# 0xWOLAND/zkvm-pairings

Hardware: AMD Instinct MI355X
Metric: BLS12-381 pairings/s on 2^20 random (G1,G2) pairs; bit-exact Gt vs ref (CPU oracle: the reference's pairings.rs is empty) (higher is better)
Workload: dtype u32

## Files before the change

### zkvm_pairings_amd/csrc/zkp_coop.hip

```cpp
#include "zkp_coop.hpp"
#include "zkp_plan.hpp"
#include "zkp_msm_plan.hpp"

#include <cstdio>
#include <cstdlib>
#include <cstring>
#include <vector>

#include "zkp_coop_prog.inc"
#include "zkp_fp28.hpp"
#include "zkp_coop_mulacc.inc"
#include "zkp_prep_dbl.inc"
#include "zkp_valid_steps.inc"

using namespace zkp28;

namespace {

constexpr int GROUPS = 5;
constexpr int LIG = ZKP_COOP_G;
constexpr int ST_SIZE = ZKP_COOP_ST_SIZE;
constexpr int NLINES = ZKP_COOP_NLINES;
static_assert(zkp::plan::NLINES == NLINES && zkp::plan::ST_SIZE == ST_SIZE && zkp::plan::GROUPS == GROUPS,
              "zkp_plan.hpp (the host's planning arithmetic, checked under sanitizers on the CPU) follows the generated programs");
// ... 6 lines not shown

struct NDev { const uint32_t* cnt; uint32_t base; };
__device__ __forceinline__ uint32_t eff_n(uint32_t n, const NDev& nd) {
    if (!nd.cnt) return n;
    const uint32_t m = *nd.cnt;
    const uint32_t left = m > nd.base ? m - nd.base : 0u;
    return left < n ? left : n;
}

struct CoopArgs {
    const uint32_t* hdr;
    const uint32_t* tbl;
    const uint4* rtbl;
    const int4* consts;
    const int4* lines;
    int4* state;
    const uint64_t* wire_in;
    uint64_t* wire_out;
    uint8_t* ok;
    int* all_ok;
    uint32_t n_checks;
    uint32_t nc;
    uint32_t k;
    uint32_t S;
    uint32_t nconst;
    uint32_t st_off;
    uint32_t chk_off;
    NDev nd;
};

__device__ __forceinline__ void lds_ld(int32_t* x, const int4* lds, int off, int S) {
// ... 162 lines not shown
                    const uint64_t* src = A.wire_in + ((size_t)check + (arg == K_WIRE2 ? A.chk_off : 0u)) * 72 + idx * 6;
                    uint64_t ww[6];
#pragma unroll
                    for (int i = 0; i < 6; i++) ww[i] = src[i];
#pragma unroll
                    for (int i = 0; i < NL; i++) {
                        const int bit = W * i, word = bit >> 6, sh = bit & 63;
                        uint64_t v = ww[word] >> sh;
                        if (sh > 64 - W && word + 1 < 6) v |= ww[word + 1] << (64 - sh);
                        x[i] = (int32_t)(v & (uint64_t)MASK);
                    }
                } else {
                    size_t rec;
                    if (arg == K_LINE) rec = ((size_t)cursor * A.k * 6 + pair6 + idx) * n_checks + check;
                    else rec = (size_t)(idx + A.st_off) * A.nc + check;
                    const int4* src = (arg == K_LINE ? A.lines : (const int4*)A.state) + rec * 4;
                    int4 v0 = src[0], v1 = src[1], v2 = src[2], v3 = src[3];
                    x[0] = v0.x; x[1] = v0.y; x[2] = v0.z; x[3] = v0.w; x[4] = v1.x; x[5] = v1.y; x[6] = v1.z; x[7] = v1.w;
                    x[8] = v2.x; x[9] = v2.y; x[10] = v2.z; x[11] = v2.w; x[12] = v3.x; x[13] = v3.y;
                }
                lds_st(lds, gbase + (int)(w & 63), PS, x);
            }
            cursor += h1;
        } else if (op == OP_GSTORE) {
            const uint32_t w = tbl[off + lig];
            const uint32_t idx = w >> 8;
            const bool part = active && ((w >> 7) & 1);
            int32_t x[NL];
            lds_ld(x, lds, gbase + (int)(w & 63), PS);
            if (arg == K_STATE) {
                if (part) {
                    int4* dst = A.state + ((size_t)(idx + A.st_off) * A.nc + check) * 4;
                    dst[0] = make_int4(x[0], x[1], x[2], x[3]);
                    dst[1] = make_int4(x[4], x[5], x[6], x[7]);
                    dst[2] = make_int4(x[8], x[9], x[10], x[11]);
                    dst[3] = make_int4(x[12], x[13], 0, 0);
                }
            } else {
                uint32_t f[NL];
                canon28(f, x);
                if (part && A.wire_out) {
                    uint64_t o[6] = {0, 0, 0, 0, 0, 0};
#pragma unroll
                    for (int i = 0; i < NL; i++) {
                        const int bit = W * i, word = bit >> 6, sh = bit & 63;
                        o[word] |= (uint64_t)f[i] << sh;
                        if (sh > 64 - W && word + 1 < 6) o[word + 1] |= (uint64_t)f[i] >> (64 - sh);
                    }
                    uint64_t* dst = A.wire_out + (size_t)check * 72 + idx * 6;
#pragma unroll
                    for (int i = 0; i < 6; i++) dst[i] = o[i];
// ... 74 lines not shown
}

__device__ __forceinline__ void ksq_forms(int32_t* xr, int32_t* xi, int32_t* yr, int32_t* yi, bool a_lane, bool v_mine) {
    if (a_lane) {
#pragma unroll
        for (int i = 0; i < NL; i++) {
            const int32_t tr = xr[i] + yr[i], ti = xi[i] + yi[i];
            const int32_t vr = v_mine ? xr[i] : yr[i], vi = v_mine ? xi[i] : yi[i];
            xr[i] = tr;
            xi[i] = ti;
            yr[i] = vi - tr;
            yi[i] = -ti - vr;
        }
    }
}
__global__ void __launch_bounds__(64, KSQ_WAVES) k_ksq(int4* state, uint32_t n_checks_in, uint32_t nc, uint32_t elem_in, uint32_t elem_snap,
                                                           uint32_t nsq, uint64_t snap_mask, NDev nd) {
    extern __shared__ int4 parked[];
    const uint32_t n_checks = eff_n(n_checks_in, nd);
    if (blockIdx.x * KS_CHECKS >= n_checks) return;
    const int lane = threadIdx.x;
    const int r = lane & 3;
    const bool b_lane = r & 1;
    const bool mine_is_v = r == 0 || r == 3;
    const uint32_t check_raw = blockIdx.x * KS_CHECKS + (lane >> 2);
    const bool active = check_raw < n_checks;
    const uint32_t check = active ? check_raw : n_checks - 1;
    const int tu = (r & 2) ? 1 : 3, tv = (r & 2) ? 5 : 2;
    int4* const st = state + (size_t)check * 4;
    auto rec = [&](uint32_t e) -> int4* { return st + (size_t)e * nc * 4; };

    int32_t xr[NL], xi[NL], yr[NL], yi[NL];
    {
        Fp28 u0, u1, v0, v1;
        rec_load(u0, rec(elem_in + 2 * tu));
        rec_load(u1, rec(elem_in + 2 * tu + 1));
        rec_load(v0, rec(elem_in + 2 * tv));
        rec_load(v1, rec(elem_in + 2 * tv + 1));
        const Fp28 &m0 = mine_is_v ? v0 : u0, &m1 = mine_is_v ? v1 : u1, &o0 = mine_is_v ? u0 : v0, &o1 = mine_is_v ? u1 : v1;
        park_st(parked, lane, m0.l, m1.l);
#pragma unroll
        for (int i = 0; i < NL; i++) { xr[i] = m0.l[i]; xi[i] = m1.l[i]; yr[i] = o0.l[i]; yi[i] = o1.l[i]; }
        ksq_forms(xr, xi, yr, yi, !b_lane, r == 0);
    }
    uint32_t snap = elem_snap;
// ... 8 lines not shown
    for (uint32_t it = 0; it < nsq; it++) {
        {
            constexpr uint32_t PL[NL] = {ZKP28_P_LIMBS};
            asm volatile(ZKP_KSQ_BODY_ASM
                         : ZKP_KSQ_BODY_IO(xr, xi, yr, yi)
                         : [p0] "s"(PL[0]), [p1] "s"(PL[1]), [p2] "s"(PL[2]), [p3] "s"(PL[3]), [p4] "s"(PL[4]), [p5] "s"(PL[5]), [p6] "s"(PL[6]),
                           [p7] "s"(PL[7]), [p8] "s"(PL[8]), [p9] "s"(PL[9]), [p10] "s"(PL[10]), [p11] "s"(PL[11]), [p12] "s"(PL[12]),
                           [p13] "s"(PL[13]), [pinv] "s"(ZKP28_PINV)
                         : ZKP_KSQ_BODY_CLOBBERS);
        }
        int l_ = lane;
        asm volatile("" : "+v"(l_));
        const bool a_lane = !(l_ & 1), v_mine = (l_ & 3) == 0;
        if (it < 64 && ((snap_mask >> it) & 1)) {
            const uint32_t chk_ = blockIdx.x * KS_CHECKS + (l_ >> 2);
            int4* const st_ = state + (size_t)(chk_ < n_checks ? chk_ : n_checks - 1) * 4;
            auto rec_ = [&](uint32_t e) -> int4* { return st_ + (size_t)e * nc * 4; };
            const int tu_ = (l_ & 2) ? 1 : 3, tv_ = (l_ & 2) ? 5 : 2;
            if (chk_ < n_checks && a_lane) {
                Fp28 o;
#pragma unroll
                for (int i = 0; i < NL; i++) o.l[i] = xr[i];
                rec_store(rec_(snap + 2 * (v_mine ? tv_ : tu_)), o);
#pragma unroll
                for (int i = 0; i < NL; i++) o.l[i] = xi[i];
                rec_store(rec_(snap + 2 * (v_mine ? tv_ : tu_) + 1), o);
#pragma unroll
                for (int i = 0; i < NL; i++) o.l[i] = yr[i];
                rec_store(rec_(snap + 2 * (v_mine ? tu_ : tv_)), o);
#pragma unroll
                for (int i = 0; i < NL; i++) o.l[i] = yi[i];
                rec_store(rec_(snap + 2 * (v_mine ? tu_ : tv_) + 1), o);
// ... 787 lines not shown
    acc_mul(acc, o.l, o.l);
    Fp28 nrm;
    acc_reduce(nrm.l, acc);
    Fp28 ninv = f_inv(nrm);
    Fp28 zi = f_mul_v(c ? c_neg(p.z) : p.z, ninv);
    Fp28 zi2 = f.sqr(zi);
    Fp28 ax = f.mul(p.x, zi2), ay = f.mul(p.y, f.mul(zi2, zi));
    if (inf) { f_zero(ax); ay = f.one(); }
    if (live) {
        fp28_to_wire(out + 24 * (size_t)i + 6 * c, ax);
        fp28_to_wire(out + 24 * (size_t)i + 12 + 6 * c, ay);
        if (out_inf && c == 0) out_inf[i] = inf ? 1 : 0;
    }
}

__global__ void __launch_bounds__(64) k_batch_inv(int4* state, uint32_t n_checks_in, uint32_t nc, uint32_t Bf, uint32_t elem_n, uint32_t elem_ninv,
                                                  uint32_t count, NDev nd) {
    const uint32_t n_checks = eff_n(n_checks_in, nd);
    const uint32_t B = Bf & 0x7fffffffu;
    const bool fermat = Bf >> 31;
    const uint32_t total = n_checks * count;
    const uint32_t L = (total + B - 1) / B;
    const uint32_t i = blockIdx.x * 64 + threadIdx.x;
    if (i >= L) return;
    auto recno = [&](uint32_t idx) -> size_t { const uint32_t j = idx / n_checks; return ((size_t)j * nc + (idx - j * n_checks)) * 4; };
    int4* N = state + (size_t)elem_n * nc * 4;
    int4* I = state + (size_t)elem_ninv * nc * 4;
    Fp28 acc = f_const(K28_ONE);
    uint32_t cnt = 0;
    Fp28 e_next;
    rec_load(e_next, N + recno(i));
#pragma unroll 1
    for (uint32_t idx = i; idx < total && cnt < B; idx += L, cnt++) {
        Fp28 e = e_next;
        if (idx + L < total && cnt + 1 < B) rec_load(e_next, N + recno(idx + L));
        if (B > 1) {
            rec_store(I + recno(idx), acc);
            if (f_is_zero(e)) e = f_const(K28_ONE);
            fp28_mul(acc, acc, e);
        } else {
            acc = e;
        }
// ... 13 lines not shown
        if (j) {
            const size_t nx = recno(i + (j - 1) * L);
            rec_load(e_next, N + nx);
            rec_load(pre_next, I + nx);
        }
        if (f_is_zero(e)) {
            f_zero(r);
        } else {
            fp28_mul(r, inv, pre);
            fp28_mul(inv, inv, e);
        }
        rec_store(I + at, r);
    }
}

__global__ void __launch_bounds__(64, 2) k_kdec_a(int4* state, uint32_t n_checks_in, uint32_t nc, uint32_t elem_snap, uint32_t count, uint32_t elem_n,
                                                  NDev nd) {
    const uint32_t n_checks = eff_n(n_checks_in, nd);
    if (blockIdx.x * 32u >= n_checks * count) return;
    const uint32_t tid = blockIdx.x * 64 + threadIdx.x;
    const int c = (int)(tid & 1);
    uint32_t e = tid >> 1;
    bool live = e < n_checks * count;
    if (!live) e = n_checks * count - 1;
    const uint32_t sn = e / n_checks, check = e - sn * n_checks;
    int4* const st = state + (size_t)check * 4;
    const uint32_t base = elem_snap + 12 * sn;
    auto rec = [&](uint32_t el) -> int4* { return st + (size_t)el * nc * 4; };
    F2 f{c};
    Fp28 z2, z3, z4, z5;
    rec_load(z2, rec(base + 6 + c));
    rec_load(z3, rec(base + 4 + c));
    rec_load(z4, rec(base + 2 + c));
    rec_load(z5, rec(base + 10 + c));
    const bool z2_zero = f.is_zero(z2);
    Fp28 s5 = f.sqr(z5), o;
    swap_pair(o, s5);
    Fp28 na = c ? c_add(o, s5) : c_sub(s5, o);
    Fp28 s4 = f.sqr(z4);
    na = c_sub(c_add(na, c_add(c_dbl(s4), s4)), c_dbl(z3));
    Fp28 nb = na;
    if (__any(z2_zero)) nb = c_dbl(f.mul(z4, z5));
    Fp28 N = z2_zero ? nb : na, D = z2_zero ? z3 : z2;
    swap_pair(o, D);
    Acc acc;
    acc_zero(acc);
    acc_mul(acc, D.l, D.l);
    acc_mul(acc, o.l, o.l);
    Fp28 n;
    acc_reduce(n.l, acc);
    if (!z2_zero) n = c_dbl(c_dbl(n));
    if (live) {
        int4* dn = rec(base + 8 + c);
        dn[0] = make_int4(N.l[0], N.l[1], N.l[2], N.l[3]);
        dn[1] = make_int4(N.l[4], N.l[5], N.l[6], N.l[7]);
        dn[2] = make_int4(N.l[8], N.l[9], N.l[10], N.l[11]);
        dn[3] = make_int4(N.l[12], N.l[13], z2_zero ? 1 : 0, 0);
        if (c == 0) rec_store(rec(elem_n + sn), n);
    }
}
__global__ void __launch_bounds__(64, 3) k_kdec_b(int4* state, uint32_t n_checks_in, uint32_t nc, uint32_t elem_snap, uint32_t count, uint32_t elem_ninv,
                                                  NDev nd) {
    const uint32_t n_checks = eff_n(n_checks_in, nd);
    if (blockIdx.x * 32u >= n_checks * count) return;
    const uint32_t tid = blockIdx.x * 64 + threadIdx.x;
    const int c = (int)(tid & 1);
    uint32_t e = tid >> 1;
    bool live = e < n_checks * count;
    if (!live) e = n_checks * count - 1;
    const uint32_t sn = e / n_checks, check = e - sn * n_checks;
    int4* const st = state + (size_t)check * 4;
    const uint32_t base = elem_snap + 12 * sn;
    auto rec = [&](uint32_t el) -> int4* { return st + (size_t)el * nc * 4; };
    F2 f{c};
    Fp28 N, D, ninv, z2, z3;
    int d_is_z3;
    {
        const int4* sn_ = rec(base + 8 + c);
        const int4 v0 = sn_[0], v1 = sn_[1], v2 = sn_[2], v3 = sn_[3];
        N.l[0] = v0.x; N.l[1] = v0.y; N.l[2] = v0.z; N.l[3] = v0.w; N.l[4] = v1.x; N.l[5] = v1.y; N.l[6] = v1.z; N.l[7] = v1.w;
        N.l[8] = v2.x; N.l[9] = v2.y; N.l[10] = v2.z; N.l[11] = v2.w; N.l[12] = v3.x; N.l[13] = v3.y;
        d_is_z3 = v3.z;
    }
    rec_load(z2, rec(base + 6 + c));
    rec_load(ninv, rec(elem_ninv + sn));
    D = z2;
    if (__any(d_is_z3 != 0)) {
        Fp28 z3e;
        rec_load(z3e, rec(base + 4 + c));
#pragma unroll
        for (int i = 0; i < NL; i++) D.l[i] = d_is_z3 ? z3e.l[i] : z2.l[i];
    }
    Fp28 dinv = f_mul_v(c ? c_neg(D) : D, ninv);
    Fp28 z1 = f.mul(N, dinv);
    Fp28 t;
    {
        Acc acc;
        acc_zero(acc);
        auto mulacc = [&](const Fp28& a, const Fp28& b, int k) {
            Fp28 ao, bo;
            swap_pair(ao, a);
            swap_pair(bo, b);
            int32_t x1[NL], x2[NL];
#pragma unroll
// ... 5 lines not shown
            acc_mul(acc, x2, bo.l);
        };
        {
            Fp28 o1;
            swap_pair(o1, z1);
            int32_t x[NL], y[NL];
#pragma unroll
            for (int i = 0; i < NL; i++) {
                x[i] = 2 * (o1.l[i] + (c ? o1.l[i] : z1.l[i]));
                y[i] = z1.l[i] - (c ? 0 : o1.l[i]);
            }
            acc_mul(acc, x, y);
        }
        {
            Fp28 z5;
            rec_load(z5, rec(base + 10 + c));
            mulacc(z2, z5, 1);
        }
        {
            Fp28 z4;
            rec_load(z3, rec(base + 4 + c));
            rec_load(z4, rec(base + 2 + c));
            mulacc(z3, z4, -3);
        }
        acc_reduce(t.l, acc);
    }
    Fp28 o;
    swap_pair(o, t);
    Fp28 z0 = c ? c_add(o, t) : c_add(c_sub(t, o), f_const(K28_ONE));
    z0 = f_vred(z0);
    if (live) {
        rec_store(rec(base + c), z0);
        rec_store(rec(base + 8 + c), z1);
    }
}

__global__ void k_fp28_op(int op, const uint64_t* a, const uint64_t* b, size_t n, uint64_t* out) {
    size_t i = (size_t)blockIdx.x * blockDim.x + threadIdx.x;
    if (i >= n) return;
    Fp28 x, y, r;
    fp28_from_wire(x, a + 6 * i);
    if (op <= 2) fp28_from_wire(y, b + 6 * i);
    switch (op) {
        case 0: fp28_mul(r, x, y); break;
        case 1: f_add(r, x, y); break;
        case 2: f_sub(r, x, y); break;
        case 3: r = c_neg(x); break;
        case 4: fp28_mul(r, x, x); break;
// ... 348 lines not shown
        if (out_inf && c == 0) out_inf[sg] = inf ? 1 : 0;
    }
}

__global__ void __launch_bounds__(64) k_primer() {}

}

namespace zkp {

struct CoopProgDev { uint32_t* hdr; uint32_t* tbl; uint4* rtbl; uint32_t nslot; uint32_t nconst; uint32_t wide; };
constexpr int MAX_PIPES = plan::MAX_PIPES;
struct CoopDev;
struct CoopPipe {
    int4* lines;  size_t lines_bytes;
    int4* state;  size_t state_bytes;
    hipStream_t stream;
    hipEvent_t done;
    CoopDev* owner;
    NDev nd;
};
struct CoopDev {
    CoopProgDev progs[ZKP_PROG_COUNT];
    int4* consts;
    CoopPipe pipe[MAX_PIPES];
    plan::Knobs kn;
    bool inv_fermat;
    int cus;
    bool prime_now;
    int prime;
    int4* big_state;
    size_t big_state_bytes;
    int4* vscratch;
    size_t vscratch_bytes;
    hipEvent_t ready;
    struct ProfEv { int cls; hipEvent_t a, b; };
    std::vector<ProfEv>* prof;
    bool prof_phase_c;
    const uint32_t* n_dev;
};

enum { PRIME_PREP, PRIME_KSQ, PRIME_INV };
enum { PROF_PREP = 0, PROF_MILLER, PROF_FEXP_A, PROF_INV, PROF_KSQ, PROF_KDEC_A, PROF_KDEC_B, PROF_C_DEEP, PROF_C_PLAIN, PROF_CLASSES };
struct ProfScope {
    CoopDev* d; hipStream_t s; hipEvent_t b = nullptr;
    ProfScope(CoopDev* d_, hipStream_t s_, int cls) : d(d_), s(s_) {
// ... 103 lines not shown
    if (d->vscratch) (void)hipFree(d->vscratch);
    for (int i = 0; i < MAX_PIPES; i++) {
        if (d->pipe[i].lines) (void)hipFree(d->pipe[i].lines);
        if (d->pipe[i].state) (void)hipFree(d->pipe[i].state);
        if (d->pipe[i].stream) (void)hipStreamDestroy(d->pipe[i].stream);
        if (d->pipe[i].done) (void)hipEventDestroy(d->pipe[i].done);
    }
    if (d->ready) (void)hipEventDestroy(d->ready);
    delete d;
    st->d_prog = nullptr;
    st->available = false;
}

bool coop_selected(const CoopState* st, int kind) { return st->available && kind != 1; }

static hipError_t ensure_buf(int4** p, size_t* cap, size_t bytes) {
    if (bytes <= *cap) return hipSuccess;
    if (*p) { hipError_t e = hipFree(*p); if (e != hipSuccess) return e; *p = nullptr; *cap = 0; }
    hipError_t e = hipMalloc((void**)p, bytes);
    if (e == hipSuccess) { *cap = bytes; zkp_dbg_alloc("coop.buf", *p, bytes); }
    return e;
}

static hipError_t prime(const CoopDev* d, hipStream_t s, size_t blocks, int cls) {
    if (!d || !d->prime || d->cus <= 0 || !blocks || !d->prime_now) return hipSuccess;
    const size_t c = (size_t)d->cus;
    const bool band = cls == PRIME_KSQ ? (blocks > 3 * c && blocks <= 4 * c) || (blocks > 6 * c && blocks <= 8 * c)
                                       : (blocks > 2 * c && blocks <= 3 * c);
    if (!(band || (d->prime >= 2 && blocks > c && blocks <= 12 * c))) return hipSuccess;
    hipLaunchKernelGGL(k_primer, dim3((unsigned)blocks), dim3(64), 0, s);
    return hipGetLastError();
// ... 102 lines not shown
                return e;
        }
    }
    return hipSuccess;
}

template <class Body>
static hipError_t for_chunks(CoopDev* d, size_t n_total, size_t k, bool need_lines, bool need_state, hipStream_t s, Body body, size_t chunk_override = 0) {
    if (!n_total) return hipSuccess;
    hipError_t e;
    const plan::Chunks pc = plan::plan_chunks(d->kn, n_total, k, need_lines, chunk_override, d->prof != nullptr);
    const size_t chunk = pc.chunk;
    const int pipes = pc.pipes;
    for (int i = 0; i < pipes; i++) {
        if (need_lines && (e = ensure_buf(&d->pipe[i].lines, &d->pipe[i].lines_bytes, plan::lines_bytes(plan::group_size(d->kn, k), pc.cmax))) != hipSuccess) return e;
        if (need_state && (e = ensure_buf(&d->pipe[i].state, &d->pipe[i].state_bytes, plan::state_bytes(pc.cmax))) != hipSuccess) return e;
    }
    if ((e = hipEventRecord(d->ready, s)) != hipSuccess) return e;
    for (int i = 0; i < pipes; i++)
        if ((e = hipStreamWaitEvent(d->pipe[i].stream, d->ready, 0)) != hipSuccess) return e;
    int c = 0;
    for (size_t base = 0; base < n_total; base += chunk, c++) {
        uint32_t n = (uint32_t)((n_total - base) < chunk ? (n_total - base) : chunk);
        if ((e = body(&d->pipe[c % pipes], base, n)) != hipSuccess) return e;
    }
    for (int i = 0; i < pipes; i++) {
        if ((e = hipEventRecord(d->pipe[i].done, d->pipe[i].stream)) != hipSuccess) return e;
        if ((e = hipStreamWaitEvent(s, d->pipe[i].done, 0)) != hipSuccess) return e;
    }
    return hipSuccess;
}

hipError_t coop_miller(CoopState* st, const uint64_t* g1, const uint64_t* g2, const uint8_t* i1, const uint8_t* i2, size_t n_checks, size_t k,
                       uint64_t* out, hipStream_t s) {
    CoopDev* d = (CoopDev*)st->d_prog;
    if (!coop_supports_k(k)) return hipErrorNotSupported;
    d->prime_now = n_checks <= d->kn.chunk;
    return for_chunks(d, n_checks, k, true, true, s, [&](CoopPipe* pp, size_t base, uint32_t n) -> hipError_t {
        return miller_on_pipe(d, pp, g1, g2, i1, i2, base, n, n, k, out + 72 * base);
    });
}

static hipError_t run_ksq(hipStream_t s, int4* state, uint32_t n_checks, uint32_t nc, uint32_t elem_in, uint32_t elem_snap, uint32_t nsq,
                          uint64_t snap_mask, CoopDev* d = nullptr, NDev nd = NDev{nullptr, 0}) {
    if (!n_checks || !nsq) return hipSuccess;
    if (snap_mask && nsq > 64) return hipErrorInvalidValue;
    { hipError_t ep = prime(d, s, (n_checks + KS_CHECKS - 1) / KS_CHECKS, PRIME_KSQ); if (ep != hipSuccess) return ep; }
    ProfScope prof(d, s, PROF_KSQ);
    hipLaunchKernelGGL(k_ksq, dim3((n_checks + KS_CHECKS - 1) / KS_CHECKS), dim3(64), 7 * 64 * sizeof(int4), s, state, n_checks, nc, elem_in, elem_snap, nsq, snap_mask, nd);
    return hipGetLastError();
}

static hipError_t run_inv(CoopDev* d, hipStream_t s, int4* state, uint32_t n, uint32_t nc, uint32_t elem_n, uint32_t elem_ninv, uint32_t count,
                          NDev nd = NDev{nullptr, 0}) {
    const size_t total = (size_t)n * count;
    if (!total) return hipSuccess;
    const plan::Inv pi = plan::plan_inv(d->kn, n, count);
    const uint32_t B = pi.batch;
    const size_t lanes = pi.lanes;
    { hipError_t ep = prime(d, s, (lanes + 63) / 64, PRIME_INV); if (ep != hipSuccess) return ep; }
    ProfScope prof(d, s, PROF_INV);
    hipLaunchKernelGGL(k_batch_inv, dim3((unsigned)((lanes + 63) / 64)), dim3(64), 0, s, state, n, nc, B | (d->inv_fermat ? 0x80000000u : 0u), elem_n,
                       elem_ninv, count, nd);
    return hipGetLastError();
}

static hipError_t run_fexp_c(CoopDev* d, CoopPipe* pp, uint32_t n, uint32_t nc, uint64_t* wire_out, uint8_t* ok, int* all_ok) {
    hipError_t e;
// ... 26 lines not shown
                e = hipErrorInvalidValue;
        }
        if (e != hipSuccess) break;
    }
    d->prof_phase_c = false;
    return e;
}

template <class PhaseA>
static hipError_t two_phase(CoopDev* d, size_t n_total, size_t k, bool need_lines, hipStream_t s, uint64_t* out, uint8_t* ok, int* all_ok,
                            PhaseA phase_a) {
    hipError_t e;
    for (size_t sb = 0; sb < n_total; sb += d->kn.super) {
        const size_t ns = n_total - sb < d->kn.super ? n_total - sb : d->kn.super;
        d->prime_now = ns <= d->kn.chunk && n_total <= d->kn.chunk;
        if ((e = ensure_buf(&d->big_state, &d->big_state_bytes, plan::state_bytes(ns))) != hipSuccess) return e;
        e = for_chunks(d, ns, k, need_lines, false, s, [&](CoopPipe* pp, size_t base, uint32_t n) -> hipError_t {
            CoopPipe v = *pp;
            v.state = d->big_state + 4 * base;
            v.nd = NDev{d->n_dev, (uint32_t)(sb + base)};
            return phase_a(&v, sb + base, n, (uint32_t)ns);
        });
        if (e != hipSuccess) return e;
        if ((e = run_inv(d, s, d->big_state, (uint32_t)ns, (uint32_t)ns, ZKP_COOP_ST_N, ZKP_COOP_ST_NINV, 1, NDev{d->n_dev, (uint32_t)sb})) != hipSuccess) return e;
        const plan::PhaseC pcc = plan::plan_phase_c(d->kn, ns, d->prof != nullptr);
        if (pcc.mode == plan::C_PARTS) {
            const size_t part = pcc.part;
            e = for_chunks(d, ns, 1, false, false, s, [&](CoopPipe* pp, size_t base, uint32_t n) -> hipError_t {
                CoopPipe v = *pp;
                v.state = d->big_state + 4 * base;
                v.nd = NDev{d->n_dev, (uint32_t)(sb + base)};
                return run_fexp_c(d, &v, n, (uint32_t)ns, out ? out + 72 * (sb + base) : nullptr, ok ? ok + sb + base : nullptr, all_ok);
            }, part);
        } else {
            CoopPipe v = d->pipe[0];
            v.state = d->big_state;
            v.stream = s;
            v.nd = NDev{d->n_dev, (uint32_t)sb};
            e = run_fexp_c(d, &v, (uint32_t)ns, (uint32_t)ns, out ? out + 72 * sb : nullptr, ok ? ok + sb : nullptr, all_ok);
        }
        if (e != hipSuccess) return e;
    }
    return hipSuccess;
}

// ... 70 lines not shown
            int one = -1, pa = -1, pb = -1;
            switch (op) {
                case 13: pa = ZKP_PROG_TW_FP2_INV_A; pb = ZKP_PROG_TW_FP2_INV_B; break;
                case 14: one = ZKP_PROG_TW_FP2_NR; break;
                case 15: one = ZKP_PROG_TW_FP2_MULFP; break;
                case 16: one = ZKP_PROG_TW_FP6_BY1; break;
                case 17: one = ZKP_PROG_TW_FP6_BY01; break;
                case 18: one = ZKP_PROG_TW_FP6_NR; break;
                case 19: pa = ZKP_PROG_TW_FP6_INV_A; pb = ZKP_PROG_TW_FP6_INV_B; break;
                default: pa = ZKP_PROG_FEXP_A_WIRE; pb = ZKP_PROG_TW_FP12_INV_B; break;
            }
            if (one >= 0) {
                if ((e = run_prog(d, &v, one, m, m, 1, ab + 72 * base, out + 72 * base, nullptr, nullptr, 0, (uint32_t)n)) != hipSuccess) return e;
                continue;
            }
            if ((e = ensure_buf(&d->pipe[0].state, &d->pipe[0].state_bytes, plan::state_bytes(d->kn.chunk))) != hipSuccess) return e;
            v.state = d->pipe[0].state;
            if ((e = run_prog(d, &v, pa, m, m, 1, ab + 72 * base, nullptr, nullptr, nullptr)) != hipSuccess) return e;
            if ((e = run_inv(d, s, v.state, m, m, ZKP_COOP_ST_N, ZKP_COOP_ST_NINV, 1)) != hipSuccess) return e;
            if ((e = run_prog(d, &v, pb, m, m, 1, nullptr, out + 72 * base, nullptr, nullptr)) != hipSuccess) return e;
            continue;
        }
        if (op <= 10) {
            if ((e = run_prog(d, &v, progs[op], m, m, 1, ab + 72 * base, out + 72 * base, nullptr, nullptr, 0, (uint32_t)n)) != hipSuccess) return e;
            if (op == 4 && (e = hipMemset2DAsync(out + 72 * base + 36, 576, 0, 288, m, s)) != hipSuccess) return e;
            continue;
        }
        if (op == 11 && (repeat < 1 || repeat > 64)) return hipErrorInvalidValue;
        if ((e = ensure_buf(&d->pipe[0].state, &d->pipe[0].state_bytes, plan::state_bytes(d->kn.chunk))) != hipSuccess) return e;
        v.state = d->pipe[0].state;
        if (op == 12) {
            if ((e = run_prog(d, &v, ZKP_PROG_TW_TO_SNAP, m, m, 1, ab + 72 * base, nullptr, nullptr, nullptr)) != hipSuccess) return e;
        } else {
            if ((e = run_prog(d, &v, ZKP_PROG_TW_TO_STATE, m, m, 1, ab + 72 * base, nullptr, nullptr, nullptr)) != hipSuccess) return e;
            if ((e = run_ksq(s, v.state, m, m, 0, ZKP_COOP_ST_SNAP, repeat, 1ull << (repeat - 1), d)) != hipSuccess) return e;
        }
        hipLaunchKernelGGL(k_kdec_a, dim3((2 * m + 63) / 64), dim3(64), 0, s, v.state, m, m, (uint32_t)ZKP_COOP_ST_SNAP, 1u, (uint32_t)ZKP_COOP_ST_KN, NDev{nullptr, 0});
        if ((e = hipGetLastError()) != hipSuccess) return e;
        if ((e = run_inv(d, s, v.state, m, m, ZKP_COOP_ST_KN, ZKP_COOP_ST_KNINV, 1)) != hipSuccess) return e;
        hipLaunchKernelGGL(k_kdec_b, dim3((2 * m + 63) / 64), dim3(64), 0, s, v.state, m, m, (uint32_t)ZKP_COOP_ST_SNAP, 1u, (uint32_t)ZKP_COOP_ST_KNINV, NDev{nullptr, 0});
        if ((e = hipGetLastError()) != hipSuccess) return e;
        if ((e = run_prog(d, &v, ZKP_PROG_TW_FROM_SNAP, m, m, 1, nullptr, out + 72 * base, nullptr, nullptr)) != hipSuccess) return e;
    }
    return hipSuccess;
}

hipError_t coop_time_prog(CoopState* st, int which, size_t n, hipStream_t s, hipEvent_t e0, hipEvent_t e1, float* ms) {
    CoopDev* d = (CoopDev*)st->d_prog;
    static const int ids[9] = {ZKP_PROG_TIME_T1, ZKP_PROG_TIME_T3, ZKP_PROG_TIME_T3E, ZKP_PROG_TIME_T6, ZKP_PROG_TIME_T12, ZKP_PROG_TIME_LIN,
                               ZKP_PROG_TIME_CYC, ZKP_PROG_TIME_CYCSD, ZKP_PROG_TIME_FILL};
    static const int ids2[3] = {ZKP_PROG_TIME_T6S, ZKP_PROG_TIME_T12S, ZKP_PROG_TIME_T12B};
    if (which < 0 || which > 19 || !n || n > 0x7fffffffu || ((which == 10 || which == 11 || which == 15) && n > d->kn.chunk)) return hipErrorInvalidValue;
    hipError_t e = ensure_buf(&d->pipe[0].state, &d->pipe[0].state_bytes, (size_t)ST_SIZE * n * 64);
    if (e != hipSuccess) return e;
    if ((which == 10 || which == 11 || which == 15) && (e = ensure_buf(&d->pipe[0].lines, &d->pipe[0].lines_bytes, (size_t)NLINES * 6 * n * 64)) != hipSuccess) return e;
    CoopPipe v = d->pipe[0];
    v.stream = s;
    bool timed = false;
    auto once = [&]() -> hipError_t {
        if (which == 9) return run_ksq(s, v.state, (uint32_t)n, (uint32_t)n, 0, 12, 400, 0);
        if (which >= 16 && which <= 19) {
            if (!timed) {
                timed = true;
                if (which == 17) return hipStreamSynchronize(s);
                if (which == 18) return run_ksq(s, v.state, (uint32_t)n, (uint32_t)n, 0, 12, 1, 0);
                hipError_t e1 = run_prog(d, &v, ZKP_PROG_TIME_T1, (uint32_t)n, (uint32_t)n, 1, nullptr, nullptr, nullptr, nullptr);
                if (e1 != hipSuccess || which == 16) return e1;
                return run_ksq(s, v.state, (uint32_t)n, (uint32_t)n, 0, 12, 1, 0);
            }
            return run_ksq(s, v.state, (uint32_t)n, (uint32_t)n, 0, 12, 57, 0);
        }
        if (which >= 12 && which <= 14) return run_prog(d, &v, ids2[which - 12], (uint32_t)n, (uint32_t)n, 1, nullptr, nullptr, nullptr, nullptr);
        if (which == 10 || which == 15) {
            const uint64_t* zero = (const uint64_t*)v.state;
            return prep(&v, zero, zero + 12 * n, nullptr, nullptr, 0, (uint32_t)n, 1, 0, 1, which == 10);
        }
        if (which == 11) return run_prog(d, &v, ZKP_PROG_MILLER1_STATE, (uint32_t)n, (uint32_t)n, 1, nullptr, nullptr, nullptr, nullptr);
        return run_prog(d, &v, ids[which], (uint32_t)n, (uint32_t)n, 1, nullptr, nullptr, nullptr, nullptr);
    };
    if (which != 11 && (e = hipMemsetAsync(v.state, 0, (size_t)ST_SIZE * n * 64, s)) != hipSuccess) return e;
    if ((e = once()) != hipSuccess) return e;
    if ((e = hipEventRecord(e0, s)) != hipSuccess) return e;
    if ((e = once()) != hipSuccess) return e;
    if ((e = hipEventRecord(e1, s)) != hipSuccess) return e;
    if ((e = hipEventSynchronize(e1)) != hipSuccess) return e;
    return hipEventElapsedTime(ms, e0, e1);
}

static bool valid_generic_only() {
    static const bool v = getenv("ZKP_VALID_GENERIC") && atoi(getenv("ZKP_VALID_GENERIC")) != 0;
    return v;
}
hipError_t coop_g1_valid(const uint64_t* g1, const uint8_t* inf, size_t n, uint8_t* status, hipStream_t s) {
    if (!n) return hipSuccess;
    if (!valid_generic_only()) {
// ... 115 lines not shown
```

### zkvm_pairings_amd/csrc/zkp_fp28.hpp

```cpp
#pragma once
#include <hip/hip_runtime.h>
#include <stdint.h>

#include "zkp_constants28.h"

namespace zkp28 {

constexpr int NL = 14;
constexpr int W = 28;
constexpr int32_t MASK = (1 << W) - 1;

struct Fp28 { int32_t l[NL]; };
struct Acc { int64_t c[2 * NL]; };

__device__ __constant__ const int32_t K28_P[NL] = {ZKP28_P_LIMBS};
#define ZKP28_DECL(name, ...) __device__ __constant__ const int32_t K28_##name[14] = {__VA_ARGS__};
ZKP28_CONST_LIST(ZKP28_DECL)
#undef ZKP28_DECL

__device__ __forceinline__ void acc_zero(Acc& a) {
#pragma unroll
    for (int i = 0; i < 2 * NL; i++) a.c[i] = 0;
}

// ... 52 lines not shown
    }
    out[NL - 1] = (int32_t)col;
}

__device__ __forceinline__ void weak_norm(int32_t* x) {
    int32_t c[NL];
#pragma unroll
    for (int i = 0; i < NL - 1; i++) {
        c[i] = (x[i] + (1 << (W - 1))) >> W;
        x[i] -= c[i] << W;
    }
#pragma unroll
    for (int i = 1; i < NL; i++) x[i] += c[i - 1];
}

__device__ __forceinline__ void fp28_mul(Fp28& r, const Fp28& a, const Fp28& b) {
    Acc acc;
    acc_zero(acc);
    acc_mul(acc, a.l, b.l);
    acc_reduce(r.l, acc);
}

__device__ __forceinline__ void fp28_from_wire(Fp28& r, const uint64_t* src) {
    uint64_t w[6];
#pragma unroll
    for (int i = 0; i < 6; i++) w[i] = src[i];
    Fp28 t;
#pragma unroll
    for (int i = 0; i < NL; i++) {
        int bit = W * i, word = bit >> 6, sh = bit & 63;
// ... 54 lines not shown
```

### zkvm_pairings_amd/csrc/zkp_plan.hpp

```cpp
#pragma once
#include <stddef.h>
#include <stdint.h>

namespace zkp {
namespace plan {

constexpr uint32_t NLINES = 68;
constexpr uint32_t ST_SIZE = 208;
constexpr uint32_t REC_BYTES = 64;
constexpr uint32_t GROUPS = 5;
constexpr uint32_t KS_CHECKS = 16;
constexpr size_t MAX_GROUP = 8;
constexpr size_t MAX_STREAM = 16;
constexpr size_t MAX_STREAM_LIMIT = 64;
constexpr size_t MIN_CHUNK = 320, MAX_CHUNK = (size_t)1 << 20, MAX_SUPER = (size_t)1 << 22;
constexpr int MAX_PIPES = 4;
constexpr size_t VALID_CHUNK = (size_t)1 << 22;

constexpr bool too_many(size_t n, size_t k = 1) { return n > 0x7fffffffu || k > 0xffffu || (k && n > 0x7fffffffu / k); }

struct Knobs {
    int n_pipes = 2;
    size_t chunk = (size_t)1 << 16;
    size_t super = (size_t)1 << 20;
// ... 15 lines not shown
    if (k.inv_batch < 1) k.inv_batch = 1;
    if (k.inv_batch > 4096) k.inv_batch = 4096;
    if (k.inv_lanes < 1) k.inv_lanes = 1;
    if (k.max_stream < MAX_GROUP) k.max_stream = MAX_GROUP;
    if (k.max_stream > MAX_STREAM_LIMIT) k.max_stream = MAX_STREAM_LIMIT;
    if (k.c_split < 0) k.c_split = 0;
    if (k.c_split > 64) k.c_split = 64;
    if (k.split_min < 1) k.split_min = 1;
    return k;
}

inline size_t group_size(const Knobs& kn, size_t k) { return k <= MAX_GROUP ? k : (k < kn.max_stream ? k : kn.max_stream); }

inline size_t lines_bytes(size_t pairs_per_group, size_t checks) { return (size_t)NLINES * pairs_per_group * 6 * checks * REC_BYTES; }
inline size_t state_bytes(size_t checks) { return (size_t)ST_SIZE * checks * REC_BYTES; }
inline size_t vscratch_bytes(size_t points) { return ((2 * points + 63) / 64) * 64 * 8 * 16; }

inline size_t blocks_coop(size_t checks) { return (checks + GROUPS - 1) / GROUPS; }
inline size_t blocks_ksq(size_t checks) { return (checks + KS_CHECKS - 1) / KS_CHECKS; }
inline size_t blocks_two_lanes(size_t units) { return (2 * units + 63) / 64; }
inline size_t blocks_one_lane(size_t units) { return (units + 63) / 64; }

struct Chunks {
    size_t chunk;
    size_t n_chunks;
    int pipes;
    size_t cmax;
};
inline Chunks plan_chunks(const Knobs& kn, size_t n_total, size_t k, bool need_lines, size_t chunk_override, bool profiling) {
    Chunks c{};
// ... 57 lines not shown
```

Before: 4.500 million.

## Pack state records to 56 bytes instead of 64-byte padded int4 records

Changes the state workspace record from four int4 (64 bytes, 2 padding words) to a packed 14-limb struct of 56 bytes, loaded and stored with 4-byte-aligned vector types. The kdec flag that used the padding word is now folded into the low bit of the top limb. The aim is to cut state memory traffic and footprint by an eighth. In exchange the accesses lose 16-byte alignment, which may split vector loads, and the flag encoding assumes the top limb has a spare bit.

```diff
diff --git a/zkvm_pairings_amd/csrc/zkp_coop.hip b/zkvm_pairings_amd/csrc/zkp_coop.hip
--- a/zkvm_pairings_amd/csrc/zkp_coop.hip
+++ b/zkvm_pairings_amd/csrc/zkp_coop.hip
@@ -44,7 +44,7 @@
     const uint4* rtbl;
     const int4* consts;
     const int4* lines;
-    int4* state;
+    Rec* state;
     const uint64_t* wire_in;
     uint64_t* wire_out;
     uint8_t* ok;
@@ -237,10 +237,13 @@
                     size_t rec;
                     if (arg == K_LINE) rec = ((size_t)cursor * A.k * 6 + pair6 + idx) * n_checks + check;
                     else rec = (size_t)(idx + A.st_off) * A.nc + check;
-                    const int4* src = (arg == K_LINE ? A.lines : (const int4*)A.state) + rec * 4;
-                    int4 v0 = src[0], v1 = src[1], v2 = src[2], v3 = src[3];
-                    x[0] = v0.x; x[1] = v0.y; x[2] = v0.z; x[3] = v0.w; x[4] = v1.x; x[5] = v1.y; x[6] = v1.z; x[7] = v1.w;
-                    x[8] = v2.x; x[9] = v2.y; x[10] = v2.z; x[11] = v2.w; x[12] = v3.x; x[13] = v3.y;
+                    if (arg == K_LINE) {
+                        const int4* src = A.lines + rec * 4;
+                        int4 v0 = src[0], v1 = src[1], v2 = src[2], v3 = src[3];
+                        x[0] = v0.x; x[1] = v0.y; x[2] = v0.z; x[3] = v0.w; x[4] = v1.x; x[5] = v1.y; x[6] = v1.z; x[7] = v1.w;
+                        x[8] = v2.x; x[9] = v2.y; x[10] = v2.z; x[11] = v2.w; x[12] = v3.x; x[13] = v3.y;
+                    } else
+                        rec_load(x, (const Rec*)A.state + rec);
                 }
                 lds_st(lds, gbase + (int)(w & 63), PS, x);
             }
@@ -253,11 +256,7 @@
             lds_ld(x, lds, gbase + (int)(w & 63), PS);
             if (arg == K_STATE) {
                 if (part) {
-                    int4* dst = A.state + ((size_t)(idx + A.st_off) * A.nc + check) * 4;
-                    dst[0] = make_int4(x[0], x[1], x[2], x[3]);
-                    dst[1] = make_int4(x[4], x[5], x[6], x[7]);
-                    dst[2] = make_int4(x[8], x[9], x[10], x[11]);
-                    dst[3] = make_int4(x[12], x[13], 0, 0);
+                    rec_store(A.state + ((size_t)(idx + A.st_off) * A.nc + check), x);
                 }
             } else {
                 uint32_t f[NL];
@@ -362,7 +361,7 @@
         }
     }
 }
-__global__ void __launch_bounds__(64, KSQ_WAVES) k_ksq(int4* state, uint32_t n_checks_in, uint32_t nc, uint32_t elem_in, uint32_t elem_snap,
+__global__ void __launch_bounds__(64, KSQ_WAVES) k_ksq(Rec* state, uint32_t n_checks_in, uint32_t nc, uint32_t elem_in, uint32_t elem_snap,
                                                            uint32_t nsq, uint64_t snap_mask, NDev nd) {
     extern __shared__ int4 parked[];
     const uint32_t n_checks = eff_n(n_checks_in, nd);
@@ -375,8 +374,8 @@
     const bool active = check_raw < n_checks;
     const uint32_t check = active ? check_raw : n_checks - 1;
     const int tu = (r & 2) ? 1 : 3, tv = (r & 2) ? 5 : 2;
-    int4* const st = state + (size_t)check * 4;
-    auto rec = [&](uint32_t e) -> int4* { return st + (size_t)e * nc * 4; };
+    Rec* const st = state + (size_t)check;
+    auto rec = [&](uint32_t e) -> Rec* { return st + (size_t)e * nc; };
 
     int32_t xr[NL], xi[NL], yr[NL], yi[NL];
     {
@@ -415,8 +414,8 @@
         const bool a_lane = !(l_ & 1), v_mine = (l_ & 3) == 0;
         if (it < 64 && ((snap_mask >> it) & 1)) {
             const uint32_t chk_ = blockIdx.x * KS_CHECKS + (l_ >> 2);
-            int4* const st_ = state + (size_t)(chk_ < n_checks ? chk_ : n_checks - 1) * 4;
-            auto rec_ = [&](uint32_t e) -> int4* { return st_ + (size_t)e * nc * 4; };
+            Rec* const st_ = state + (size_t)(chk_ < n_checks ? chk_ : n_checks - 1);
+            auto rec_ = [&](uint32_t e) -> Rec* { return st_ + (size_t)e * nc; };
             const int tu_ = (l_ & 2) ? 1 : 3, tv_ = (l_ & 2) ? 5 : 2;
             if (chk_ < n_checks && a_lane) {
                 Fp28 o;
@@ -1234,7 +1233,7 @@
     }
 }
 
-__global__ void __launch_bounds__(64) k_batch_inv(int4* state, uint32_t n_checks_in, uint32_t nc, uint32_t Bf, uint32_t elem_n, uint32_t elem_ninv,
+__global__ void __launch_bounds__(64) k_batch_inv(Rec* state, uint32_t n_checks_in, uint32_t nc, uint32_t Bf, uint32_t elem_n, uint32_t elem_ninv,
                                                   uint32_t count, NDev nd) {
     const uint32_t n_checks = eff_n(n_checks_in, nd);
     const uint32_t B = Bf & 0x7fffffffu;
@@ -1243,9 +1242,9 @@
     const uint32_t L = (total + B - 1) / B;
     const uint32_t i = blockIdx.x * 64 + threadIdx.x;
     if (i >= L) return;
-    auto recno = [&](uint32_t idx) -> size_t { const uint32_t j = idx / n_checks; return ((size_t)j * nc + (idx - j * n_checks)) * 4; };
-    int4* N = state + (size_t)elem_n * nc * 4;
-    int4* I = state + (size_t)elem_ninv * nc * 4;
+    auto recno = [&](uint32_t idx) -> size_t { const uint32_t j = idx / n_checks; return (size_t)j * nc + (idx - j * n_checks); };
+    Rec* N = state + (size_t)elem_n * nc;
+    Rec* I = state + (size_t)elem_ninv * nc;
     Fp28 acc = f_const(K28_ONE);
     uint32_t cnt = 0;
     Fp28 e_next;
@@ -1289,7 +1288,7 @@
     }
 }
 
-__global__ void __launch_bounds__(64, 2) k_kdec_a(int4* state, uint32_t n_checks_in, uint32_t nc, uint32_t elem_snap, uint32_t count, uint32_t elem_n,
+__global__ void __launch_bounds__(64, 2) k_kdec_a(Rec* state, uint32_t n_checks_in, uint32_t nc, uint32_t elem_snap, uint32_t count, uint32_t elem_n,
                                                   NDev nd) {
     const uint32_t n_checks = eff_n(n_checks_in, nd);
     if (blockIdx.x * 32u >= n_checks * count) return;
@@ -1299,9 +1298,9 @@
     bool live = e < n_checks * count;
     if (!live) e = n_checks * count - 1;
     const uint32_t sn = e / n_checks, check = e - sn * n_checks;
-    int4* const st = state + (size_t)check * 4;
+    Rec* const st = state + (size_t)check;
     const uint32_t base = elem_snap + 12 * sn;
-    auto rec = [&](uint32_t el) -> int4* { return st + (size_t)el * nc * 4; };
+    auto rec = [&](uint32_t el) -> Rec* { return st + (size_t)el * nc; };
     F2 f{c};
     Fp28 z2, z3, z4, z5;
     rec_load(z2, rec(base + 6 + c));
@@ -1326,15 +1325,12 @@
     acc_reduce(n.l, acc);
     if (!z2_zero) n = c_dbl(c_dbl(n));
     if (live) {
-        int4* dn = rec(base + 8 + c);
-        dn[0] = make_int4(N.l[0], N.l[1], N.l[2], N.l[3]);
-        dn[1] = make_int4(N.l[4], N.l[5], N.l[6], N.l[7]);
-        dn[2] = make_int4(N.l[8], N.l[9], N.l[10], N.l[11]);
-        dn[3] = make_int4(N.l[12], N.l[13], z2_zero ? 1 : 0, 0);
+        N.l[NL - 1] = (int32_t)((uint32_t)N.l[NL - 1] << 1) | (z2_zero ? 1 : 0);
+        rec_store(rec(base + 8 + c), N);
         if (c == 0) rec_store(rec(elem_n + sn), n);
     }
 }
-__global__ void __launch_bounds__(64, 3) k_kdec_b(int4* state, uint32_t n_checks_in, uint32_t nc, uint32_t elem_snap, uint32_t count, uint32_t elem_ninv,
+__global__ void __launch_bounds__(64, 3) k_kdec_b(Rec* state, uint32_t n_checks_in, uint32_t nc, uint32_t elem_snap, uint32_t count, uint32_t elem_ninv,
                                                   NDev nd) {
     const uint32_t n_checks = eff_n(n_checks_in, nd);
     if (blockIdx.x * 32u >= n_checks * count) return;
@@ -1344,25 +1340,24 @@
     bool live = e < n_checks * count;
     if (!live) e = n_checks * count - 1;
     const uint32_t sn = e / n_checks, check = e - sn * n_checks;
-    int4* const st = state + (size_t)check * 4;
+    Rec* const st = state + (size_t)check;
     const uint32_t base = elem_snap + 12 * sn;
-    auto rec = [&](uint32_t el) -> int4* { return st + (size_t)el * nc * 4; };
+    Rec* const r0 = st + (size_t)(base + c) * nc;
+    auto rec = [&](uint32_t el) -> Rec* { return r0 + (size_t)el * nc; };
     F2 f{c};
     Fp28 N, D, ninv, z2, z3;
     int d_is_z3;
     {
-        const int4* sn_ = rec(base + 8 + c);
-        const int4 v0 = sn_[0], v1 = sn_[1], v2 = sn_[2], v3 = sn_[3];
-        N.l[0] = v0.x; N.l[1] = v0.y; N.l[2] = v0.z; N.l[3] = v0.w; N.l[4] = v1.x; N.l[5] = v1.y; N.l[6] = v1.z; N.l[7] = v1.w;
-        N.l[8] = v2.x; N.l[9] = v2.y; N.l[10] = v2.z; N.l[11] = v2.w; N.l[12] = v3.x; N.l[13] = v3.y;
-        d_is_z3 = v3.z;
-    }
-    rec_load(z2, rec(base + 6 + c));
-    rec_load(ninv, rec(elem_ninv + sn));
+        rec_load(N, rec(8));
+        d_is_z3 = N.l[NL - 1] & 1;
+        N.l[NL - 1] >>= 1;
+    }
+    rec_load(z2, rec(6));
+    rec_load(ninv, (st + (size_t)(elem_ninv + sn) * nc));
     D = z2;
     if (__any(d_is_z3 != 0)) {
         Fp28 z3e;
-        rec_load(z3e, rec(base + 4 + c));
+        rec_load(z3e, rec(4));
 #pragma unroll
         for (int i = 0; i < NL; i++) D.l[i] = d_is_z3 ? z3e.l[i] : z2.l[i];
     }
@@ -1398,13 +1393,13 @@
         }
         {
             Fp28 z5;
-            rec_load(z5, rec(base + 10 + c));
+            rec_load(z5, rec(10));
             mulacc(z2, z5, 1);
         }
         {
             Fp28 z4;
-            rec_load(z3, rec(base + 4 + c));
-            rec_load(z4, rec(base + 2 + c));
+            rec_load(z3, rec(4));
+            rec_load(z4, rec(2));
             mulacc(z3, z4, -3);
         }
         acc_reduce(t.l, acc);
@@ -1414,8 +1409,12 @@
     Fp28 z0 = c ? c_add(o, t) : c_add(c_sub(t, o), f_const(K28_ONE));
     z0 = f_vred(z0);
     if (live) {
-        rec_store(rec(base + c), z0);
-        rec_store(rec(base + 8 + c), z1);
+        uint32_t l_ = __builtin_amdgcn_mbcnt_hi(~0u, __builtin_amdgcn_mbcnt_lo(~0u, 0u));
+        asm volatile("" : "+v"(l_));
+        const uint32_t e_ = (blockIdx.x * 64 + l_) >> 1, sn_ = e_ / n_checks;
+        Rec* const w0 = state + ((size_t)(elem_snap + 12 * sn_ + (l_ & 1)) * nc + (e_ - sn_ * n_checks));
+        rec_store(w0, z0);
+        rec_store(w0 + (size_t)8 * nc, z1);
     }
 }
 
@@ -1794,7 +1793,7 @@
 struct CoopDev;
 struct CoopPipe {
     int4* lines;  size_t lines_bytes;
-    int4* state;  size_t state_bytes;
+    Rec* state;  size_t state_bytes;
     hipStream_t stream;
     hipEvent_t done;
     CoopDev* owner;
@@ -1809,7 +1808,7 @@
     int cus;
     bool prime_now;
     int prime;
-    int4* big_state;
+    Rec* big_state;
     size_t big_state_bytes;
     int4* vscratch;
     size_t vscratch_bytes;
@@ -1943,7 +1942,8 @@
 
 bool coop_selected(const CoopState* st, int kind) { return st->available && kind != 1; }
 
-static hipError_t ensure_buf(int4** p, size_t* cap, size_t bytes) {
+template <class T>
+static hipError_t ensure_buf(T** p, size_t* cap, size_t bytes) {
     if (bytes <= *cap) return hipSuccess;
     if (*p) { hipError_t e = hipFree(*p); if (e != hipSuccess) return e; *p = nullptr; *cap = 0; }
     hipError_t e = hipMalloc((void**)p, bytes);
@@ -2076,7 +2076,7 @@
     const int pipes = pc.pipes;
     for (int i = 0; i < pipes; i++) {
         if (need_lines && (e = ensure_buf(&d->pipe[i].lines, &d->pipe[i].lines_bytes, plan::lines_bytes(plan::group_size(d->kn, k), pc.cmax))) != hipSuccess) return e;
-        if (need_state && (e = ensure_buf(&d->pipe[i].state, &d->pipe[i].state_bytes, plan::state_bytes(pc.cmax))) != hipSuccess) return e;
+        if (need_state && (e = ensure_buf(&d->pipe[i].state, &d->pipe[i].state_bytes, plan::state_ws_bytes(pc.cmax))) != hipSuccess) return e;
     }
     if ((e = hipEventRecord(d->ready, s)) != hipSuccess) return e;
     for (int i = 0; i < pipes; i++)
@@ -2103,7 +2103,7 @@
     });
 }
 
-static hipError_t run_ksq(hipStream_t s, int4* state, uint32_t n_checks, uint32_t nc, uint32_t elem_in, uint32_t elem_snap, uint32_t nsq,
+static hipError_t run_ksq(hipStream_t s, Rec* state, uint32_t n_checks, uint32_t nc, uint32_t elem_in, uint32_t elem_snap, uint32_t nsq,
                           uint64_t snap_mask, CoopDev* d = nullptr, NDev nd = NDev{nullptr, 0}) {
     if (!n_checks || !nsq) return hipSuccess;
     if (snap_mask && nsq > 64) return hipErrorInvalidValue;
@@ -2113,7 +2113,7 @@
     return hipGetLastError();
 }
 
-static hipError_t run_inv(CoopDev* d, hipStream_t s, int4* state, uint32_t n, uint32_t nc, uint32_t elem_n, uint32_t elem_ninv, uint32_t count,
+static hipError_t run_inv(CoopDev* d, hipStream_t s, Rec* state, uint32_t n, uint32_t nc, uint32_t elem_n, uint32_t elem_ninv, uint32_t count,
                           NDev nd = NDev{nullptr, 0}) {
     const size_t total = (size_t)n * count;
     if (!total) return hipSuccess;
@@ -2170,10 +2170,10 @@
     for (size_t sb = 0; sb < n_total; sb += d->kn.super) {
         const size_t ns = n_total - sb < d->kn.super ? n_total - sb : d->kn.super;
         d->prime_now = ns <= d->kn.chunk && n_total <= d->kn.chunk;
-        if ((e = ensure_buf(&d->big_state, &d->big_state_bytes, plan::state_bytes(ns))) != hipSuccess) return e;
+        if ((e = ensure_buf(&d->big_state, &d->big_state_bytes, plan::state_ws_bytes(ns))) != hipSuccess) return e;
         e = for_chunks(d, ns, k, need_lines, false, s, [&](CoopPipe* pp, size_t base, uint32_t n) -> hipError_t {
             CoopPipe v = *pp;
-            v.state = d->big_state + 4 * base;
+            v.state = d->big_state + base;
             v.nd = NDev{d->n_dev, (uint32_t)(sb + base)};
             return phase_a(&v, sb + base, n, (uint32_t)ns);
         });
@@ -2184,7 +2184,7 @@
             const size_t part = pcc.part;
             e = for_chunks(d, ns, 1, false, false, s, [&](CoopPipe* pp, size_t base, uint32_t n) -> hipError_t {
                 CoopPipe v = *pp;
-                v.state = d->big_state + 4 * base;
+                v.state = d->big_state + base;
                 v.nd = NDev{d->n_dev, (uint32_t)(sb + base)};
                 return run_fexp_c(d, &v, n, (uint32_t)ns, out ? out + 72 * (sb + base) : nullptr, ok ? ok + sb + base : nullptr, all_ok);
             }, part);
@@ -2285,7 +2285,7 @@
                 if ((e = run_prog(d, &v, one, m, m, 1, ab + 72 * base, out + 72 * base, nullptr, nullptr, 0, (uint32_t)n)) != hipSuccess) return e;
                 continue;
             }
-            if ((e = ensure_buf(&d->pipe[0].state, &d->pipe[0].state_bytes, plan::state_bytes(d->kn.chunk))) != hipSuccess) return e;
+            if ((e = ensure_buf(&d->pipe[0].state, &d->pipe[0].state_bytes, plan::state_ws_bytes(d->kn.chunk))) != hipSuccess) return e;
             v.state = d->pipe[0].state;
             if ((e = run_prog(d, &v, pa, m, m, 1, ab + 72 * base, nullptr, nullptr, nullptr)) != hipSuccess) return e;
             if ((e = run_inv(d, s, v.state, m, m, ZKP_COOP_ST_N, ZKP_COOP_ST_NINV, 1)) != hipSuccess) return e;
@@ -2298,7 +2298,7 @@
             continue;
         }
         if (op == 11 && (repeat < 1 || repeat > 64)) return hipErrorInvalidValue;
-        if ((e = ensure_buf(&d->pipe[0].state, &d->pipe[0].state_bytes, plan::state_bytes(d->kn.chunk))) != hipSuccess) return e;
+        if ((e = ensure_buf(&d->pipe[0].state, &d->pipe[0].state_bytes, plan::state_ws_bytes(d->kn.chunk))) != hipSuccess) return e;
         v.state = d->pipe[0].state;
         if (op == 12) {
             if ((e = run_prog(d, &v, ZKP_PROG_TW_TO_SNAP, m, m, 1, ab + 72 * base, nullptr, nullptr, nullptr)) != hipSuccess) return e;
@@ -2322,9 +2322,9 @@
                                ZKP_PROG_TIME_CYC, ZKP_PROG_TIME_CYCSD, ZKP_PROG_TIME_FILL};
     static const int ids2[3] = {ZKP_PROG_TIME_T6S, ZKP_PROG_TIME_T12S, ZKP_PROG_TIME_T12B};
     if (which < 0 || which > 19 || !n || n > 0x7fffffffu || ((which == 10 || which == 11 || which == 15) && n > d->kn.chunk)) return hipErrorInvalidValue;
-    hipError_t e = ensure_buf(&d->pipe[0].state, &d->pipe[0].state_bytes, (size_t)ST_SIZE * n * 64);
+    hipError_t e = ensure_buf(&d->pipe[0].state, &d->pipe[0].state_bytes, plan::state_ws_bytes(n));
     if (e != hipSuccess) return e;
-    if ((which == 10 || which == 11 || which == 15) && (e = ensure_buf(&d->pipe[0].lines, &d->pipe[0].lines_bytes, (size_t)NLINES * 6 * n * 64)) != hipSuccess) return e;
+    if ((which == 10 || which == 11 || which == 15) && (e = ensure_buf(&d->pipe[0].lines, &d->pipe[0].lines_bytes, plan::lines_bytes(1, n))) != hipSuccess) return e;
     CoopPipe v = d->pipe[0];
     v.stream = s;
     bool timed = false;
@@ -2349,7 +2349,7 @@
         if (which == 11) return run_prog(d, &v, ZKP_PROG_MILLER1_STATE, (uint32_t)n, (uint32_t)n, 1, nullptr, nullptr, nullptr, nullptr);
         return run_prog(d, &v, ids[which], (uint32_t)n, (uint32_t)n, 1, nullptr, nullptr, nullptr, nullptr);
     };
-    if (which != 11 && (e = hipMemsetAsync(v.state, 0, (size_t)ST_SIZE * n * 64, s)) != hipSuccess) return e;
+    if (which != 11 && (e = hipMemsetAsync(v.state, 0, plan::state_ws_bytes(n), s)) != hipSuccess) return e;
     if ((e = once()) != hipSuccess) return e;
     if ((e = hipEventRecord(e0, s)) != hipSuccess) return e;
     if ((e = once()) != hipSuccess) return e;
diff --git a/zkvm_pairings_amd/csrc/zkp_fp28.hpp b/zkvm_pairings_amd/csrc/zkp_fp28.hpp
--- a/zkvm_pairings_amd/csrc/zkp_fp28.hpp
+++ b/zkvm_pairings_amd/csrc/zkp_fp28.hpp
@@ -3,6 +3,7 @@
 #include <stdint.h>
 
 #include "zkp_constants28.h"
+#include "zkp_plan.hpp"
 
 namespace zkp28 {
 
@@ -90,6 +91,29 @@
     for (int i = 1; i < NL; i++) x[i] += c[i - 1];
 }
 
+struct Rec { int32_t l[NL]; };
+static_assert(sizeof(Rec) == zkp::plan::STATE_REC_BYTES && alignof(Rec) == 4 && NL == (int)zkp::plan::STATE_REC_LIMBS, "one state record geometry: zkp_plan.hpp");
+typedef int32_t rec_q4_ __attribute__((ext_vector_type(4)));
+typedef int32_t rec_q2_ __attribute__((ext_vector_type(2)));
+typedef rec_q4_ rec_q4 __attribute__((aligned(4)));
+typedef rec_q2_ rec_q2 __attribute__((aligned(4)));
+__device__ __forceinline__ void rec_store(Rec* dst, const int32_t* x) {
+    rec_q4* d = (rec_q4*)dst;
+    d[0] = rec_q4{x[0], x[1], x[2], x[3]};
+    d[1] = rec_q4{x[4], x[5], x[6], x[7]};
+    d[2] = rec_q4{x[8], x[9], x[10], x[11]};
+    *(rec_q2*)(d + 3) = rec_q2{x[12], x[13]};
+}
+__device__ __forceinline__ void rec_load(int32_t* x, const Rec* src) {
+    const rec_q4* s = (const rec_q4*)src;
+    const rec_q4 v0 = s[0], v1 = s[1], v2 = s[2];
+    const rec_q2 v3 = *(const rec_q2*)(s + 3);
+    x[0] = v0.x; x[1] = v0.y; x[2] = v0.z; x[3] = v0.w; x[4] = v1.x; x[5] = v1.y; x[6] = v1.z; x[7] = v1.w;
+    x[8] = v2.x; x[9] = v2.y; x[10] = v2.z; x[11] = v2.w; x[12] = v3.x; x[13] = v3.y;
+}
+__device__ __forceinline__ void rec_store(Rec* dst, const Fp28& x) { rec_store(dst, x.l); }
+__device__ __forceinline__ void rec_load(Fp28& x, const Rec* src) { rec_load(x.l, src); }
+
 __device__ __forceinline__ void fp28_mul(Fp28& r, const Fp28& a, const Fp28& b) {
     Acc acc;
     acc_zero(acc);
diff --git a/zkvm_pairings_amd/csrc/zkp_plan.hpp b/zkvm_pairings_amd/csrc/zkp_plan.hpp
--- a/zkvm_pairings_amd/csrc/zkp_plan.hpp
+++ b/zkvm_pairings_amd/csrc/zkp_plan.hpp
@@ -8,6 +8,8 @@
 constexpr uint32_t NLINES = 68;
 constexpr uint32_t ST_SIZE = 208;
 constexpr uint32_t REC_BYTES = 64;
+constexpr uint32_t STATE_REC_LIMBS = 14;
+constexpr uint32_t STATE_REC_BYTES = 4 * STATE_REC_LIMBS;
 constexpr uint32_t GROUPS = 5;
 constexpr uint32_t KS_CHECKS = 16;
 constexpr size_t MAX_GROUP = 8;
@@ -53,6 +55,7 @@
 
 inline size_t lines_bytes(size_t pairs_per_group, size_t checks) { return (size_t)NLINES * pairs_per_group * 6 * checks * REC_BYTES; }
 inline size_t state_bytes(size_t checks) { return (size_t)ST_SIZE * checks * REC_BYTES; }
+inline size_t state_ws_bytes(size_t checks) { return (size_t)ST_SIZE * checks * STATE_REC_BYTES; }
 inline size_t vscratch_bytes(size_t points) { return ((2 * points + 63) / 64) * 64 * 8 * 16; }
 
 inline size_t blocks_coop(size_t checks) { return (checks + GROUPS - 1) / GROUPS; }
```

Result: no change. 4.507 million, median of 5 (+0.2%).
